# driskai/scenario_gym

Measured on AMD Instinct MI355X. Metric: entity-steps/sec (batched rollout), higher is better.
Workload: dtype f64

## Files before the change

### scenario_gym_amd/csrc/sgym_control.hpp

```cpp
#pragma once

namespace sg {

struct CtlLds { double ctrl[9][64]; double seg[5][64]; };

template <bool FAST, bool RIDERS = false>
__device__ __forceinline__ void control_body_l(CtlLds &lds ,
                                               const unsigned qblock ,
                                               const Params &p, double timestep, int n_steps, int first, int k0,
                                               const double *actions , double *tab, int row0, int metrics)
{
    const int lane = threadIdx.x;
    const size_t q = (size_t)qblock * 64 + lane;
    const int ent_raw = p.ctl_ent[q];
    const bool active = ent_raw >= 0;
    const uint32_t ent = active ? (uint32_t)ent_raw : 0u;
    const uint32_t r = ent / (uint32_t)p.EP;
    const LanePtr st(p.stat + (size_t)(ent >> 6) * (ST_COUNT * 64), (ent & 63) * 8u);
    const LanePtr dy(p.dyn + (size_t)(ent >> 6) * ((size_t)p.FROWS * 64), (ent & 63) * 8u);
    const int64_t meta = fld<int64_t>(st, ST_META);
    const int kind = active ? (int)(meta & 0xff) : SG_KIND_NONE;
    const double min_t = fld(st, ST_MIN_T), bl = fld(st, ST_BL);
    const bool is_ego = active && (int)(ent - r * (uint32_t)p.EP) == p.sstat[r].ego;
#pragma unroll
    for (int c = 0; c < 9; ++c) lds.ctrl[c][lane] = fld(st, ST_CTRL + c);
    const size_t NP = (size_t)p.n_ctl_pad;
    double *cst = p.ctl_state + q;

    double pose[6], t, prev_t;
    double m_avg, m_max, m_t;
    bool present;
    CtrlState cs;
    if (first) {
        const sg_scenario_state &sd = p.sdyn[r];
        t = sd.t;
        prev_t = sd.prev_t;
        m_avg = sd.ego_avg_speed; m_max = sd.ego_max_speed; m_t = sd.avg_t;
        present = fld<uint64_t>(dy, SG_F_PRESENT) != 0;
#pragma unroll
        for (int c = 0; c < 6; ++c) pose[c] = fld(dy, SG_F_POSE + c);
        cs.speed = fld(dy, SG_F_CTRL + 0); cs.e_lon_prev = fld(dy, SG_F_CTRL + 1);
        cs.e_lat_prev = fld(dy, SG_F_CTRL + 2); cs.e_lon_int = fld(dy, SG_F_CTRL + 3);
    } else {
#pragma unroll
        for (int c = 0; c < 6; ++c) pose[c] = cst[(CS_POSE + c) * NP];
        present = cst[CS_PRESENT * NP] != 0.0;
        cs.speed = cst[(CS_CTRL + 0) * NP]; cs.e_lon_prev = cst[(CS_CTRL + 1) * NP];
        cs.e_lat_prev = cst[(CS_CTRL + 2) * NP]; cs.e_lon_int = cst[(CS_CTRL + 3) * NP];
        t = cst[CS_T * NP];
        prev_t = cst[CS_PREV_T * NP];
        m_avg = cst[(CS_METRIC + 0) * NP]; m_max = cst[(CS_METRIC + 1) * NP]; m_t = cst[(CS_METRIC + 2) * NP];
    }
    if (!active) present = false;

    Table T;
    {
        const double *kn = p.knots + fld<int64_t>(st, ST_KNOT_OFF) * 7;
        T.x = kn; T.xs = 7; T.y = kn + 1; T.ys = 7; T.cs = 1;
        T.n = active ? (int)(meta >> 32) : 0;
    }
    double seg_hi;
    int seg_cur;
    double sgr[5] = {0.0, 0.0, 0.0, 0.0, 0.0};
    auto seg_publish = [&](const Segment &S) {
        lds.seg[0][lane] = S.x_lo;
        lds.seg[1][lane] = S.ylo[0]; lds.seg[2][lane] = S.ylo[1];
        lds.seg[3][lane] = S.sl[0]; lds.seg[4][lane] = S.sl[1];
        if (FAST) { sgr[0] = S.x_lo; sgr[1] = S.ylo[0]; sgr[2] = S.ylo[1]; sgr[3] = S.sl[0]; sgr[4] = S.sl[1]; }
        seg_hi = S.x_hi;
        seg_cur = S.cur;
    };
    {
        Segment S;
        S.cur = seg_locate(T, t);
        seg_load(T, S);
        seg_publish(S);
    }
    double *out = tab + (q * (size_t)(p.tab_steps + 1) + (size_t)row0) * CT_W;
    double *out1 = out + (size_t)p.n_ctl_pad * ((size_t)(p.tab_steps + 1) * CT_W);
    double *out2 = out1 + (size_t)p.n_ctl_pad * ((size_t)(p.tab_steps + 1) * CT_W);
    const bool replay_lane = RIDERS && (kind == SG_KIND_REPLAY || kind == SG_KIND_AGENT_REPLAY);
    const double max_t = fld(st, ST_MAX_T);
    const bool is_static = (int)(meta >> 32) == 1;
    Table TR{};
    Segment SR{};
    if (RIDERS) {
        TR = lane_table(p, replay_lane ? kind : SG_KIND_NONE, p.sstat[r], (int)(ent - r * (uint32_t)p.EP), st);
        if (!replay_lane) TR.n = 0;
        SR.cur = seg_locate(TR, t);
        seg_load(TR, SR);
    }
    sg_loads_done();
    const bool fast_kind = FAST && !p.ctl_general && sg_all(!active || (kind == SG_KIND_AGENT_PID && bl > 0.0 && bl < 0x1p400));
    const RecipDiv rd_l(active ? bl : 1.0), rd_10(10.0);
    double cpr[9];
#pragma unroll
    for (int c = 0; c < 9; ++c) cpr[c] = FAST ? fld(st, ST_CTRL + c) : 0.0;
    sg_loads_done();

    for (int k = 0; k < n_steps; ++k) {
        const double *Kp = SG_TRIG;
        if (!FAST) asm volatile("" : "+s"(Kp));
        ConstTbl K = (ConstTbl)Kp;
        const double next_t = t + timestep;
        const double state_dt = t - prev_t;
        const double dt = next_t - t;
        if (FAST && fast_kind && sg_all(!active || (present && !(next_t > seg_hi) && __builtin_fabs(pose[3]) < 1.0e5))) {
            const double dq = next_t - sgr[0];
            const double tx = sgr[3] * dq + sgr[1], ty = sgr[4] * dq + sgr[2];
            double sin_h, cos_h;
            sg_sincos_core(pose[3], sin_h, cos_h, K);
            const double e0 = tx - pose[0], e1 = ty - pose[1];
            const double e_lon = cos_h * e0 + sin_h * e1;
            const double e_lat = -sin_h * e0 + cos_h * e1;
            const double speed0 = cs.speed;
            const double g_mid = 1.0 - rd_10.div(0.9 * (speed0 - 5.0));
            const double gain = (speed0 > 5.0 && speed0 <= 15) ? g_mid : (speed0 > 15 ? 0.1 : 1.0);
            const RecipDiv rd(state_dt);
            const double d_lat = e_lat - cs.e_lat_prev, d_lon = e_lon - cs.e_lon_prev;
            const double e_lat_D = rd.div(d_lat);
            const double kp = cpr[SG_C_STEER_KP] * gain, kd = cpr[SG_C_STEER_KD] * gain;
            double steer = kp * e_lat + kd * e_lat_D;
            const double e_lon_D = rd.div(d_lon);
            const double e_lon_I = cs.e_lon_int + e_lon * state_dt;
            double accel = cpr[SG_C_ACCEL_KP] * e_lon + cpr[SG_C_ACCEL_KD] * e_lon_D + cpr[SG_C_ACCEL_KI] * e_lon_I;
            accel = __builtin_fabs(e_lon) > 0.1 ? accel : 0.0;
            const double max_steer = cpr[SG_C_MAX_STEER], max_accel = cpr[SG_C_MAX_ACCEL];
            const double max_speed = cpr[SG_C_MAX_SPEED], allow_rev = cpr[SG_C_ALLOW_REVERSE];
            accel = __builtin_fmin(__builtin_fmax(accel, -max_accel), max_accel);
            steer = __builtin_fmin(__builtin_fmax(steer, -max_steer), max_steer);
            const double dxs = speed0 * cos_h, dys = speed0 * sin_h;
            double tan_s = sg_tan_poly(steer, K);
            const bool steep = !(__builtin_fabs(steer) < 0.67434);
            if (sg_any(steep & active)) {
                double s2, c2;
                sg_sincos_core(steer, s2, c2, K);
                tan_s = steep ? s2 / c2 : tan_s;
            }
            const double hnum = speed0 * tan_s;
            const double dh = hnum == 0.0 ? hnum : rd_l.div(hnum);
            const double nx = pose[0] + dxs * dt, ny = pose[1] + dys * dt, nh = pose[3] + dh * dt;
            double nspeed = speed0 + accel * dt;
            nspeed = allow_rev == 0.0 ? __builtin_fmax(0.0, nspeed) : nspeed;
            nspeed = max_speed == max_speed ? __builtin_fmin(max_speed, nspeed) : nspeed;
            bool ok = rd.safe(d_lat) & rd.safe(d_lon) & (__builtin_fabs(steer) < 1.0e5) & (rd_l.safe(hnum) | (hnum == 0.0));
            double n_avg = m_avg, n_max = m_max, n_mt = m_t;
            if (metrics) {
                const RecipDiv rdt(dt), rnt(next_t);
                const double ax = nx - pose[0], ay = ny - pose[1];
                const double az = pose[2] - pose[2];
                const double speed = sg_norm3(rdt.div(ax), rdt.div(ay), 0.0);
                const double w = rnt.div(m_t);
                n_avg = m_avg + (1.0 - w) * (speed - m_avg);
                n_max = __builtin_fmax(speed, m_max);
                n_mt = next_t;
                ok = ok & (!is_ego | (rdt.safe(ax) & rdt.safe(ay) & rnt.safe(m_t) & (dt > 0.0) & (az == 0.0)));
            }
            if (sg_all(!active || ok)) {
                cs.e_lat_prev = e_lat; cs.e_lon_prev = e_lon; cs.e_lon_int = e_lon_I; cs.speed = nspeed;
                pose[0] = nx; pose[1] = ny; pose[3] = nh;
                if (is_ego) { m_avg = n_avg; m_max = n_max; m_t = n_mt; }
                prev_t = t;
                t = next_t;
                *reinterpret_cast<double4 *>(out + (size_t)k * CT_W) = make_double4(pose[0], pose[1], pose[3], cs.speed);
                *reinterpret_cast<double4 *>(out1 + (size_t)k * CT_W) = make_double4(cs.e_lon_prev, cs.e_lat_prev, cs.e_lon_int, 0.0);
                if (is_ego && metrics) *reinterpret_cast<double4 *>(out2 + (size_t)k * CT_W) = make_double4(m_avg, m_max, m_t, 0.0);
                continue;
            }
        }
        double act_a = 0.0, act_s = 0.0;
        if (kind == SG_KIND_AGENT_VEHICLE && actions) {
            const double *a = actions + ((size_t)(k0 + k) * p.R + r) * 2;
            act_a = a[0];
            act_s = a[1];
        }
        if (next_t > seg_hi) {
            Segment S;
            S.x_hi = seg_hi;
            S.cur = seg_cur;
            seg_advance(T, S, next_t);
            seg_publish(S);
            sg_loads_done();
        }
        double np_[6];
        const double dq = next_t - lds.seg[0][lane];
        np_[0] = lds.seg[3][lane] * dq + lds.seg[1][lane];
        np_[1] = lds.seg[4][lane] * dq + lds.seg[2][lane];
        bool npres = false;
        if (RIDERS && replay_lane) {
            if (next_t > SR.x_hi) { seg_advance(TR, SR, next_t); sg_loads_done(); }
            const double dqr = next_t - SR.x_lo;
#pragma unroll
            for (int c = 0; c < 6; ++c) np_[c] = SR.sl[c] * dqr + SR.ylo[c];
            npres = kind == SG_KIND_REPLAY ? (p.persist || is_static || (next_t >= min_t && next_t <= max_t))
                                           : (present || min_t >= t);
        } else if (present) {
            npres = true;
            const double tx = np_[0], ty = np_[1];
#pragma unroll
            for (int c = 0; c < 6; ++c) np_[c] = pose[c];
            double sin_h, cos_h;
            sg_sincos(pose[3], sin_h, cos_h, K);
            auto cp = [&](int q) -> double { return lds.ctrl[q][lane]; };
            if (kind == SG_KIND_AGENT_PID)
                pid_step(cs, cp, bl, state_dt, dt, tx, ty, sin_h, cos_h, np_, K);
            else
                vehicle_step(cs, cp, bl, dt, act_a, act_s, sin_h, cos_h, np_, K);
        } else if (active && min_t >= t) {
            npres = true;
            Segment S;
            S.cur = seg_cur;
            seg_load(T, S);
            sg_loads_done();
            const double dqs = next_t - S.x_lo;
#pragma unroll
            for (int c = 0; c < 6; ++c) np_[c] = S.sl[c] * dqs + S.ylo[c];
        }
        if (is_ego && npres && metrics) {
            double prev[6];
            if (!present) {
                own_position_extrap(T.x, T.n, t, prev);
                sg_loads_done();
            } else {
#pragma unroll
                for (int c = 0; c < 6; ++c) prev[c] = pose[c];
            }
            const double v0 = (np_[0] - prev[0]) / dt, v1 = (np_[1] - prev[1]) / dt, v2 = (np_[2] - prev[2]) / dt;
            const double speed = sg_norm3(v0, v1, v2);
            const double w = m_t / next_t;
            m_avg += (1.0 - w) * (speed - m_avg);
            m_t = next_t;
            m_max = __builtin_fmax(speed, m_max);
        }
        present = npres;
        if (npres) {
#pragma unroll
            for (int c = 0; c < 6; ++c) pose[c] = np_[c];
        }
        prev_t = t;
        t = next_t;
        *reinterpret_cast<double4 *>(out + (size_t)k * CT_W) = make_double4(pose[0], pose[1], pose[3], cs.speed);
        *reinterpret_cast<double4 *>(out1 + (size_t)k * CT_W) = make_double4(cs.e_lon_prev, cs.e_lat_prev, cs.e_lon_int, 0.0);
        if (is_ego && metrics) *reinterpret_cast<double4 *>(out2 + (size_t)k * CT_W) = make_double4(m_avg, m_max, m_t, 0.0);
        if (RIDERS) *reinterpret_cast<double4 *>(out2 + (size_t)k * CT_W) = make_double4(pose[2], pose[4], pose[5], present ? 1.0 : 0.0);
    }
#pragma unroll
    for (int c = 0; c < 6; ++c) cst[(CS_POSE + c) * NP] = pose[c];
    cst[CS_PRESENT * NP] = present ? 1.0 : 0.0;
    cst[(CS_CTRL + 0) * NP] = cs.speed; cst[(CS_CTRL + 1) * NP] = cs.e_lon_prev;
    cst[(CS_CTRL + 2) * NP] = cs.e_lat_prev; cst[(CS_CTRL + 3) * NP] = cs.e_lon_int;
    cst[CS_T * NP] = t;
    cst[CS_PREV_T * NP] = prev_t;
    cst[(CS_METRIC + 0) * NP] = m_avg; cst[(CS_METRIC + 1) * NP] = m_max; cst[(CS_METRIC + 2) * NP] = m_t;
}

template <bool FAST, bool RIDERS = false>
__device__ __forceinline__ void control_body(const Params &p, double timestep, int n_steps, int first, int k0,
                                             const double *actions , double *tab, int row0, int metrics)
{
    __shared__ CtlLds lds;
    control_body_l<FAST, RIDERS>(lds, blockIdx.x, p, timestep, n_steps, first, k0, actions, tab, row0, metrics);
}

#ifdef SG_UNIT_CTL
static __global__ __launch_bounds__(64, SG_CTL_WAVES) void control_kernel(Params p, double timestep, int n_steps, int first, int k0,
                                                     const double *actions , double *tab, int row0, int metrics)
{
    control_body<false>(p, timestep, n_steps, first, k0, actions, tab, row0, metrics);
}
#endif
#ifdef SG_UNIT_CTL
static __global__ __launch_bounds__(64, 2) void control_kernel_riders(Params p, double timestep, int n_steps, int first, int k0,
                                                               const double *actions , double *tab, int row0, int metrics)
{
    control_body<false, true>(p, timestep, n_steps, first, k0, actions, tab, row0, 0);
}
#endif
#ifdef SG_UNIT_CTL
static __global__ __launch_bounds__(64, 1) void control_kernel_fast(Params p, double timestep, int n_steps, int first, int k0,
                                                             const double *actions , double *tab, int row0, int metrics)
{
#ifdef SG_CTL_SETPRIO
    __builtin_amdgcn_s_setprio(3);
#endif
    control_body<true>(p, timestep, n_steps, first, k0, actions, tab, row0, metrics);
}
#endif

}
```

### scenario_gym_amd/csrc/sgym_core.hpp

```cpp
#pragma once

namespace sg {

enum {
    ST_BW = 0, ST_BL, ST_BCX, ST_BCY,
    ST_MIN_T, ST_MAX_T,
    ST_KNOT_OFF,
    ST_META,
    ST_ROUTE,
    ST_CTL,
    ST_CTRL,
    NCTRL_ROWS = 13,
    ST_COUNT = ST_CTRL + NCTRL_ROWS
};
constexpr uint32_t ROW = 512;

struct ScenStatic {
    double t0, length;
    int64_t grid_off;
    int32_t grid_n, ego;
};

struct RoadNet { double x0, y0, inv_cell; int32_t nx, ny; int64_t cell_base; };
struct RoadCand { int32_t poly; uint32_t edge_off; uint16_t n_edges; uint8_t ref_sel, ref_inside; };
struct RoadIndex {
    const RoadNet *nets;
    const int32_t *net_of_scen;
    const uint16_t *cells;
    const uint32_t *cell_off;
    const RoadCand *cand;
    const int32_t *cand_edges;
    const double *edges;
    const uint32_t *poly_layers;
    const uint32_t *net_flags;
    const int64_t *imp_off;
    const double *imp_edges;
    const double *imp_aux;
    const double *imp_m;
    int32_t n_nets;
};

struct Params {
    int R, E, EP;
    int persist;
    unsigned term_mask;
    int rec_cap, ev_cap;
    const double *stat;
    const ScenStatic *sstat;
    const double *knots;
    const double *grid_t;
    double *grid_y;
    double *dyn;
    sg_scenario_state *sdyn;
    sg_event *events;
    double *ev_pose;
    double *ev_hpose;
    double *rec_t, *rec_pose;
    const double *routes;
    const double *gon;
    int WV, FROWS;
    sg_social_force sf;
    const int32_t *ctl_ent;
    double *ctl_state;
    int n_ctl_pad;
    const double *ext_pose;
    int32_t *rss_state, *rss_code, *rss_seen;
    double *rss_safe;
    double *rssq;
    int32_t *rssq_n;
    int32_t rssq_cap;
    const unsigned char *reset_mask;
    const RoadIndex *road;
    int ctl_general;
    int ped_serial;
    int quiet;
    int tab_steps;
    int noise_mode;
    double noise_std_lon, noise_std_lat;
    const double *noise_normals;
    long long noise_len;
    unsigned long long noise_seed;
    int ped_behaviour;
    int n_ped_models;
    const double *ped_models;
    const int32_t *model_of;
#ifdef SG_PHASE_TIMERS
    unsigned long long *phase_cycles;
#endif
};

enum { PM_BEHAVIOUR = 0, PM_SF = 1, PM_STD_LON = 13, PM_STD_LAT = 14, PM_W = 16 };
static_assert(sizeof(sg_social_force) == 12 * sizeof(double), "sg_social_force is twelve doubles");

enum { CT_X = 0, CT_Y, CT_H, CT_SPEED, CT_W = 4, CT_ELON = 0, CT_ELAT, CT_EINT, CT_MAVG = 0, CT_MMAX, CT_MT, CT_PLANES = 3 };
enum { CS_POSE = 0, CS_PRESENT = 6, CS_CTRL = 7, CS_T = 11, CS_PREV_T = 12, CS_METRIC = 13, CS_COUNT = 16 };

#define SG_GLOBAL __attribute__((address_space(1)))
struct LanePtr {
    SG_GLOBAL char *a[3];
    __device__ __forceinline__ LanePtr(const double *blk, uint32_t voff)
    {
        a[0] = (SG_GLOBAL char *)(reinterpret_cast<char *>(const_cast<double *>(blk)) + voff);
        a[1] = a[0] + 8 * ROW;
        a[2] = a[0] + 16 * ROW;
        asm("" : "+v"(a[1]), "+v"(a[2]));
    }
};
template <typename T = double>
__device__ __forceinline__ T fld(const LanePtr &lp, int f)
{
    const int b = f < 24 ? f >> 3 : 2;
    return *reinterpret_cast<SG_GLOBAL const T *>(lp.a[b] + (f - 8 * b) * (int)ROW);
}
template <typename T>
__device__ __forceinline__ void stf(const LanePtr &lp, int f, T v)
{
    const int b = f < 24 ? f >> 3 : 2;
    *reinterpret_cast<SG_GLOBAL T *>(lp.a[b] + (f - 8 * b) * (int)ROW) = v;
}

__device__ __forceinline__ double sg_norm3(double a, double b, double c)
{
    return __builtin_sqrt(__builtin_fma(c, c, __builtin_fma(b, b, a * a)));
}
__device__ __forceinline__ double sg_norm2(double a, double b)
{
    return __builtin_sqrt(__builtin_fma(b, b, a * a));
}

__device__ __noinline__ double2 sg_sincos_slow(double x)
{
    return make_double2(sin(x), cos(x));
}

static __constant__ double SG_TRIG[48] = {
    6.36619772367581382433e-01,
    1.57079632673412561417e+00,
    6.07710050630396597660e-11,
    2.02226624879595063154e-21,
    -1.66666666666666324348e-01, 8.33333333332248946124e-03, -1.98412698298579493134e-04,
    2.75573137070700676789e-06, -2.50507602534068634195e-08, 1.58969099521155010221e-10,
    4.16666666666666019037e-02, -1.38888888888741095749e-03, 2.48015872894767294178e-05,
    -2.75573143513906633035e-07, 2.08757232129817482790e-09, -1.13596475577881948265e-11,
    3.33333333333334091986e-01, 1.33333333333201242699e-01, 5.39682539762260521377e-02,
    2.18694882948595424599e-02, 8.86323982359930005737e-03, 3.59207910759131235356e-03,
    1.45620945432529025516e-03, 5.88041240820264096874e-04, 2.46463134818469906812e-04,
    7.81794442939557092300e-05, 7.14072491382608190305e-05, -1.85586374855275456654e-05,
    2.59073051863633712884e-05, 0.0, 0.0, 0.0,
    3.33333333333329318027e-01, -1.99999999998764832476e-01, 1.42857142725034663711e-01, -1.11111104054623557880e-01,
    9.09088713343650656196e-02, -7.69187620504482999495e-02, 6.66107313738753120669e-02, -5.83357013379057348645e-02,
    4.97687799461593236017e-02, -3.65315727442169155270e-02, 1.62858201153657823623e-02, 0.0, 0.0, 0.0, 0.0, 0.0,
};

typedef const __attribute__((address_space(4))) double *ConstTbl;

__device__ __forceinline__ void sg_sincos_core(double x, double &s, double &c, ConstTbl K);

__device__ __forceinline__ void sg_sincos(double x, double &s, double &c, ConstTbl K = (ConstTbl)SG_TRIG)
{
    if (!(__builtin_fabs(x) < 1.0e5)) {
        double2 sc = sg_sincos_slow(x);
        s = sc.x;
        c = sc.y;
        return;
    }
    sg_sincos_core(x, s, c, K);
}

__device__ __forceinline__ void sg_sincos_core(double x, double &s, double &c, ConstTbl K)
{
    double fn = __builtin_rint(x * K[0]);
    int n = (int)fn;
    double t = x - fn * K[1];
    double w = fn * K[2];
    double r = t - w;
    w = fn * K[3] - ((t - r) - w);
    double y0 = r - w;
    double y1 = (r - y0) - w;
    double z = y0 * y0;
    double v = z * y0;
    double rs = K[5] + z * (K[6] + z * (K[7] + z * (K[8] + z * K[9])));
    double ks = y0 - ((z * (0.5 * y1 - v * rs) - y1) - v * K[4]);
    double rc = z * (K[10] + z * (K[11] + z * (K[12] + z * (K[13] + z * (K[14] + z * K[15])))));
    double ay = __builtin_fabs(y0);
    uint64_t qb = ((uint64_t)__double_as_longlong(ay) - ((uint64_t)0x00200000 << 32)) & 0xFFFFFFFF00000000ULL;
    double qx = ay > 0.78125 ? 0.28125 : __longlong_as_double((long long)qb);
    qx = ay < 0.3 ? 0.0 : qx;
    double hz = 0.5 * z - qx;
    double a = 1.0 - qx;
    double kc = a - (hz - (z * rc - y0 * y1));
    double ss = (n & 1) ? kc : ks;
    double cc = (n & 1) ? ks : kc;
    s = (n & 2) ? -ss : ss;
    c = ((n + 1) & 2) ? -cc : cc;
}

__device__ __forceinline__ double sg_tan_poly(double x, ConstTbl K)
{
    ConstTbl T = K + 16;
    double z = x * x;
    double w = z * z;
    double r = T[1] + w * (T[3] + w * (T[5] + w * (T[7] + w * (T[9] + w * T[11]))));
    double v = z * (T[2] + w * (T[4] + w * (T[6] + w * (T[8] + w * (T[10] + w * T[12])))));
    double s = z * x;
    r = z * (s * (r + v));
    r = r + T[0] * s;
    return x + r;
}

__device__ __forceinline__ double sg_tan(double x, ConstTbl K)
{
    if (!(__builtin_fabs(x) < 0.67434)) {
        double s, c;
        sg_sincos(x, s, c, K);
        return s / c;
    }
    return sg_tan_poly(x, K);
}

#define SG_TRIG32_ERR 4.0e-6f
__device__ __forceinline__ void sg_sincos_f32(double h, float &s, float &c)
{
    if (!(__builtin_fabs(h) < 1.0e5)) {
        double2 sc = sg_sincos_slow(h);
        s = (float)sc.x;
        c = (float)sc.y;
        return;
    }
    const double rev = h * 1.59154943091895345554e-01;
    const float f = (float)(rev - __builtin_rint(rev));
    s = __builtin_amdgcn_sinf(f);
    c = __builtin_amdgcn_cosf(f);
}

__device__ __forceinline__ double sg_pred(double x)
{
    long long b = __double_as_longlong(x);
    if (x > 0.0) return __longlong_as_double(b - 1);
    if (x < 0.0) return __longlong_as_double(b + 1);
    return -4.9406564584124654e-324;
}

__device__ __forceinline__ bool sg_any(bool p) { return __builtin_amdgcn_ballot_w64(p) != 0; }
__device__ __forceinline__ bool sg_all(bool p) { return __builtin_amdgcn_ballot_w64(!p) == 0; }

__device__ __forceinline__ double shfl_d(double v, int src) { return __shfl(v, src, 64); }

__device__ __forceinline__ void sg_loads_done() { __builtin_amdgcn_s_waitcnt(0x0F70); }
__device__ __forceinline__ void sg_lgkm_done() { __builtin_amdgcn_s_waitcnt(0xC07F); }

struct RecipDiv {
    double b, r;
    bool ok;
    __device__ __forceinline__ explicit RecipDiv(double den) : b(den)
    {
        double ab = __builtin_fabs(den);
        ok = ab > 0x1p-500 && ab < 0x1p500;
        double r0 = __builtin_amdgcn_rcp(den);
        double e0 = __builtin_fma(-den, r0, 1.0);
        double r1 = __builtin_fma(r0, e0, r0);
        double e1 = __builtin_fma(-den, r1, 1.0);
        r = __builtin_fma(r1, e1, r1);
    }
    __device__ __forceinline__ bool safe(double a) const
    {
        uint32_t e = ((uint32_t)__double2hiint(a) >> 20) & 0x7ffu;
        return ok & (((e - 64u) < 1920u) | (__double_as_longlong(a) == 0));
    }
    __device__ __forceinline__ double div(double a) const
    {
        double q0 = a * r;
        double e = __builtin_fma(-b, q0, a);
        return __builtin_fma(e, r, q0);
    }
};

struct Table {
    const double *x;
    const double *y;
    int n;
    int xs, ys, cs;
    __device__ __forceinline__ double X(int i) const { return x[(size_t)i * xs]; }
    __device__ __forceinline__ double Y(int i, int c) const { return y[(size_t)i * ys + (size_t)c * cs]; }
};

struct Segment {
    double x_lo, x_hi;
    double ylo[6], sl[6];
    int cur;
};

__device__ __forceinline__ void seg_load(const Table &T, Segment &S)
{
    const int n = T.n, cur = S.cur;
    if (n <= 0) {
        S.x_lo = 0.0;
        S.x_hi = __builtin_inf();
#pragma unroll
        for (int c = 0; c < 6; ++c) { S.ylo[c] = 0.0; S.sl[c] = 0.0; }
        return;
    }
    if (cur == 0 || cur >= n || n == 1) {
        int row = cur == 0 ? 0 : n - 1;
        double x0 = T.X(row);
        S.x_lo = x0;
        S.x_hi = (cur == 0 && n > 1) ? sg_pred(x0) : __builtin_inf();
#pragma unroll
        for (int c = 0; c < 6; ++c) { S.ylo[c] = T.Y(row, c); S.sl[c] = 0.0; }
        return;
    }
    double x_lo = T.X(cur - 1), x_hi = T.X(cur);
    S.x_lo = x_lo;
    S.x_hi = x_hi;
    double dx = x_hi - x_lo;
#pragma unroll
    for (int c = 0; c < 6; ++c) {
        double a = T.Y(cur - 1, c), b = T.Y(cur, c);
        S.ylo[c] = a;
        S.sl[c] = (b - a) / dx;
    }
}

__device__ __forceinline__ int seg_locate(const Table &T, double t)
{
    const int n = T.n;
    if (n <= 1) return 0;
    if (t < T.X(0)) return 0;
    if (t > T.X(n - 1)) return n;
    int lo = 0, hi = n;
    while (lo < hi) {
        int mid = (lo + hi) >> 1;
        if (T.X(mid) < t) lo = mid + 1; else hi = mid;
    }
    return lo < 1 ? 1 : (lo > n - 1 ? n - 1 : lo);
}

__device__ __forceinline__ void seg_advance(const Table &T, Segment &S, double t)
{
    if (t > S.x_hi) {
        int cur = S.cur == 0 ? 1 : S.cur;
        while (cur <= T.n - 1 && T.X(cur) < t) ++cur;
        S.cur = cur;
        seg_load(T, S);
    }
}

__device__ __forceinline__ void own_position_extrap(const double *kn, int n, double t, double (&out)[6])
{
    if (n == 1) {
        double x_lo = kn[0];
#pragma unroll
        for (int c = 0; c < 6; ++c) {
            double slope = kn[1 + c] - kn[1 + c];
            out[c] = slope * (t - x_lo) + kn[1 + c];
        }
        return;
    }
    int lo = 0, hi = n;
    while (lo < hi) {
        int mid = (lo + hi) >> 1;
        if (kn[(size_t)mid * 7] < t) lo = mid + 1; else hi = mid;
    }
    int idx = lo < 1 ? 1 : (lo > n - 1 ? n - 1 : lo);
    const double *a = kn + (size_t)(idx - 1) * 7, *b = kn + (size_t)idx * 7;
#pragma unroll
    for (int c = 0; c < 6; ++c) {
        double slope = (b[1 + c] - a[1 + c]) / (b[0] - a[0]);
        out[c] = slope * (t - a[0]) + a[1 + c];
    }
}

__device__ __forceinline__ void sg_corners(double x, double y, double s, double c, double W, double L,
                                           double cx, double cy, double *o)
{
    double pxm = cx - 0.5 * L, pxp = cx + 0.5 * L, pyp = cy + 0.5 * W, pym = cy - 0.5 * W;
    double ns = -s;
    o[0] = x + (pxm * c + pyp * ns); o[1] = y + (pxm * s + pyp * c);
    o[2] = x + (pxp * c + pyp * ns); o[3] = y + (pxp * s + pyp * c);
    o[4] = x + (pxp * c + pym * ns); o[5] = y + (pxp * s + pym * c);
    o[6] = x + (pxm * c + pym * ns); o[7] = y + (pxm * s + pym * c);
}

__device__ __forceinline__ bool sg_sat_pass(const double *P, const double *Q)
{
    double o = (P[4] - P[0]) * (P[7] - P[3]) - (P[5] - P[1]) * (P[6] - P[2]);
    bool sep = false;
#pragma unroll
    for (int i = 0; i < 4; ++i) {
        int j = (i + 1) & 3;
        double ax = P[2 * i], ay = P[2 * i + 1];
        double ex = P[2 * j] - ax, ey = P[2 * j + 1] - ay;
        bool all_out = true;
#pragma unroll
        for (int k = 0; k < 4; ++k) {
            double cr = ex * (Q[2 * k + 1] - ay) - ey * (Q[2 * k] - ax);
            bool out = o > 0 ? (cr < 0) : (cr > 0);
            all_out = all_out && out;
        }
        sep = sep || all_out;
    }
    return sep;
}
__device__ __forceinline__ bool sg_quads_intersect(const double *A, const double *B)
{
    return !(sg_sat_pass(A, B) || sg_sat_pass(B, A));
}

typedef float v2f __attribute__((ext_vector_type(2)));
typedef double v2d __attribute__((ext_vector_type(2)));
typedef float v4f __attribute__((ext_vector_type(4)));

template <int NS, bool PED, bool CROWD = false, bool ROADTAB = false>
struct TileLds {
    float cx[NS], cy[NS];
    float2 sc[NS];
    float2 cen[NS];
    unsigned long long xtab[64][NS / 64], ytab[64][NS / 64];
    double cor[8][NS > 64 ? NS : 2];
    float2 half[NS];
    int last[NS];
    int vote[4][8];
    double ctrl[PED ? 4 : 9][NS];
    double boxwl[2][NS];
    double px[PED ? NS : 1], py[PED ? NS : 1], vx[PED ? NS : 1], vy[PED ? NS : 1];
    double ox[PED ? NS : 1], oy[PED ? NS : 1], stp[PED ? NS : 1];
    unsigned char isped[PED ? NS : 1];
    double sx[CROWD ? NS : 1], sy[CROWD ? NS : 1], ss[CROWD ? NS : 1];
    double r2hi[CROWD ? NS : 1], r2lo[CROWD ? NS : 1];
    uint32_t nq[CROWD ? 8 : 1][CROWD ? NS : 1];
    double ego_m[CROWD ? 3 : 1];
    unsigned long long ego_last[CROWD ? (NS + 63) / 64 : 1];
    int ego_nev[2];
    static constexpr bool GON = CROWD && NS != 128;
    double gon[GON ? 128 : 1];
    static constexpr bool ROAD_TAB = ROADTAB;
    static constexpr int ROAD_EDGES = 64;
    double road_tab[ROADTAB ? ROAD_EDGES * 5 : 1];
    double road_m;
    RoadNet road_net;
    int road_info[4];

    static constexpr int SLOTS = NS;
    static constexpr int SCRATCH_BYTES = NS * 40 + 64 * (NS > 64 ? NS : 2);
    static constexpr int PAIR_CAP = NS > 64 ? 320 : 128;
    __device__ __forceinline__ char *wave_scratch(int wave) { return reinterpret_cast<char *>(cx) + wave * (PAIR_CAP * 20); }
};
static_assert(TileLds<256, true>::PAIR_CAP * 20 * 4 <= TileLds<256, true>::SCRATCH_BYTES, "pair scratch");
static_assert(TileLds<128, true>::PAIR_CAP * 20 * 2 <= TileLds<128, true>::SCRATCH_BYTES, "pair scratch");
static_assert(TileLds<64, true>::PAIR_CAP * 20 <= TileLds<64, true>::SCRATCH_BYTES, "pair scratch");
typedef TileLds<256, true> TileLdsWide;
static_assert(offsetof(TileLdsWide, half) == TileLdsWide::SCRATCH_BYTES, "collision scratch is contiguous");

}
```

### scenario_gym_amd/csrc/sgym_queue.hpp

```cpp
#pragma once

namespace sg {

enum { Q_TICKET = 0, Q_HEAD = 1, Q_ERR = 2, Q_ITEMS_DONE = 3, Q_CTL_CLAIMED = 4, Q_STATE_WORDS = 8 };
constexpr int Q_SEATS = 1 << 14;
enum { Q_ERR_CTL_WAIT = 1, Q_ERR_BLOCK_WAIT = 2, Q_ERR_RING_WAIT = 3 };
constexpr int Q_MAX_CHUNKS = 255;
constexpr int Q_PROG_STRIDE = 32;

struct TabQueue {
    unsigned *state;
    unsigned *ctl_prog;
    unsigned *blk_prog;
    unsigned *chunk_cnt;
    unsigned *seats;
    long long defer_ticks;
    double *tab;
    size_t buf_doubles;
    const double *actions;
    unsigned *trace;
    unsigned long long *times;
    long long timeout_ticks;
    int n_chunks, n_buf, nblk, n_ctl_waves;
    int nap;
    int lag_prio;
    int handoff;
    int k0[Q_MAX_CHUNKS + 1];
};

__device__ __forceinline__ unsigned q_peek(const unsigned *w)
{
    return (unsigned)__builtin_amdgcn_readfirstlane((int)__hip_atomic_load(w, __ATOMIC_RELAXED, __HIP_MEMORY_SCOPE_AGENT));
}

__device__ __forceinline__ bool q_wait_ge(const unsigned *w, unsigned want, const TabQueue &tq, unsigned code)
{
    if (q_peek(w) >= want) return true;
    const long long t0 = wall_clock64();
    for (int spin = 0;; ++spin) {
        if (spin < 4) __builtin_amdgcn_s_sleep(16);
        else if (spin < 12) __builtin_amdgcn_s_sleep(112);
        else {
            const int n = min(tq.nap, 1 << min((spin - 12) >> 2, 6));
            for (int i = 0; i < n; ++i) __builtin_amdgcn_s_sleep(127);
        }
        if (q_peek(w) >= want) return true;
        if ((spin & 7) == 7 && q_peek(tq.state + Q_ERR) != 0) return false;
        if (wall_clock64() - t0 > tq.timeout_ticks) {
            if (threadIdx.x == 0) atomicCAS(tq.state + Q_ERR, 0u, code);
            return false;
        }
    }
}

__device__ __forceinline__ void q_acquire()
{
    __builtin_amdgcn_fence(__ATOMIC_ACQUIRE, "agent");
    asm volatile("s_dcache_inv\n\ts_waitcnt lgkmcnt(0)" ::: "memory");
}

__device__ __forceinline__ void q_release()
{
    asm volatile("s_waitcnt vmcnt(0)" ::: "memory");
    __builtin_amdgcn_fence(__ATOMIC_RELEASE, "agent");
    asm volatile("s_waitcnt vmcnt(0)" ::: "memory");
}

template <int G>
__device__ __forceinline__ void q_handoff_writethrough(const Params &p, unsigned b, int lane)
{
    asm volatile("s_waitcnt vmcnt(0)" ::: "memory");
    typedef SG_GLOBAL unsigned long long gu64;
    constexpr int FR = SG_F_COLL + 1;
    gu64 *rows = (gu64 *)(p.dyn + (size_t)b * ((size_t)FR * 64)) + lane;
    unsigned long long v[FR];
#pragma unroll
    for (int f = 0; f < FR; ++f) v[f] = __hip_atomic_load(rows + f * 64, __ATOMIC_RELAXED, __HIP_MEMORY_SCOPE_AGENT);
#pragma unroll
    for (int f = 0; f < FR; ++f) __hip_atomic_store(rows + f * 64, v[f], __ATOMIC_RELAXED, __HIP_MEMORY_SCOPE_AGENT);
    static_assert(sizeof(sg_scenario_state) % 8 == 0, "scenario records are copied in 8-byte words");
    constexpr int SW = (int)(sizeof(sg_scenario_state) / 8);
    const int gl = (int)b * 64 + lane, r = gl / G, slot = gl & (G - 1);
    if (r < p.R) {
        gu64 *sd = (gu64 *)(p.sdyn + r);
        for (int w = slot; w < SW; w += G) {
            const unsigned long long v = __hip_atomic_load(sd + w, __ATOMIC_RELAXED, __HIP_MEMORY_SCOPE_AGENT);
            __hip_atomic_store(sd + w, v, __ATOMIC_RELAXED, __HIP_MEMORY_SCOPE_AGENT);
        }
    }
    asm volatile("s_waitcnt vmcnt(0)" ::: "memory");
}

template <int G, unsigned F>
__device__ __forceinline__ void tabq_body(const Params &p, double timestep, int force, const TabQueue &tq)
{
    constexpr bool RSS = (F & V_RSS) != 0;
    using Tile = typename Variant<G, 1, F>::Lds;
    static_assert(sizeof(Tile) >= sizeof(CtlLds), "the pre-pass role lays its LDS over the tile");
    __shared__ Tile lds;
    __shared__ typename std::conditional<RSS, RssQueue, char>::type rssq_lds;
    const int lane = threadIdx.x;
    unsigned ticket = ~0u;
    {
        const unsigned hw = (unsigned)__builtin_amdgcn_s_getreg((4 << 0) | (0 << 6) | (31 << 11));
        const unsigned xcc = (unsigned)__builtin_amdgcn_s_getreg((20 << 0) | (0 << 6) | (3 << 11));
        const unsigned seat = ((xcc & 15u) << 10) | (((hw >> 13) & 7u) << 7) | (((hw >> 12) & 1u) << 6) | (((hw >> 8) & 15u) << 2) | ((hw >> 4) & 3u);
        unsigned rank = 0;
        if (lane == 0) {
            atomicAdd(tq.state + Q_TICKET, 1u);
            rank = atomicAdd(tq.seats + seat, 1u);
        }
        rank = (unsigned)__builtin_amdgcn_readfirstlane((int)rank);
        bool claim = rank == 0 && q_peek(tq.state + Q_CTL_CLAIMED) < (unsigned)tq.n_ctl_waves;
        if (rank != 0) {
            const long long t0 = wall_clock64();
            while (q_peek(tq.state + Q_CTL_CLAIMED) < (unsigned)tq.n_ctl_waves) {
                if (wall_clock64() - t0 > tq.defer_ticks) { claim = true; break; }
                __builtin_amdgcn_s_sleep(8);
            }
        }
        if (claim) {
            unsigned idx = 0;
            if (lane == 0) idx = atomicAdd(tq.state + Q_CTL_CLAIMED, 1u);
            idx = (unsigned)__builtin_amdgcn_readfirstlane((int)idx);
            if (idx < (unsigned)tq.n_ctl_waves) ticket = idx;
        }
    }

    if (ticket < (unsigned)tq.n_ctl_waves) {
        __builtin_amdgcn_s_setprio(3);
        CtlLds &cl = *reinterpret_cast<CtlLds *>(&lds);
        for (int c = 0; c < tq.n_chunks; ++c) {
            if (c >= tq.n_buf && !q_wait_ge(tq.chunk_cnt + (c - tq.n_buf), (unsigned)tq.nblk, tq, Q_ERR_RING_WAIT)) break;
            control_body_l<true>(cl, ticket, p, timestep, tq.k0[c + 1] - tq.k0[c], c == 0, tq.k0[c], tq.actions,
                                 tq.tab + (size_t)(c % tq.n_buf) * tq.buf_doubles, 0, RSS ? 0 : 1);
            q_release();
            if (tq.times && lane == 0) tq.times[(size_t)tq.n_chunks * tq.nblk * 4 + (size_t)ticket * tq.n_chunks + c] = wall_clock64();
            if (lane == 0) __hip_atomic_store(tq.ctl_prog + ticket * Q_PROG_STRIDE, (unsigned)(c + 1), __ATOMIC_RELAXED, __HIP_MEMORY_SCOPE_AGENT);
        }
        __builtin_amdgcn_s_setprio(0);
        if (q_peek(tq.state + Q_ERR) != 0) return;
    }

    const unsigned n_items = (unsigned)tq.n_chunks * (unsigned)tq.nblk;
    unsigned done_b = ~0u, done_c = 0;
    for (;;) {
        unsigned item = 0;
        if (lane == 0) {
            if (done_b != ~0u) {
                __hip_atomic_store(tq.blk_prog + done_b, done_c + 1, __ATOMIC_RELAXED, __HIP_MEMORY_SCOPE_AGENT);
                if (tq.n_buf < tq.n_chunks) atomicAdd(tq.chunk_cnt + done_c, 1u);
                atomicAdd(tq.state + Q_ITEMS_DONE, 1u);
            }
            item = atomicAdd(tq.state + Q_HEAD, 1u);
        }
        item = (unsigned)__builtin_amdgcn_readfirstlane((int)item);
        done_b = ~0u;
        if (item >= n_items) break;
        const unsigned c = item / (unsigned)tq.nblk, b = item - c * (unsigned)tq.nblk;
        auto trace = [&](unsigned stage) {
            if (tq.trace && lane == 0) __hip_atomic_store(tq.trace + b, (c << 8) | stage, __ATOMIC_RELAXED, __HIP_MEMORY_SCOPE_AGENT);
        };
        trace(1);
        auto stamp = [&](int k) {
            if (tq.times && lane == 0) tq.times[(size_t)item * 4 + k] = wall_clock64();
        };
        stamp(0);
        if (tq.lag_prio) __builtin_amdgcn_s_setprio(0);
        const bool behind = c != 0 && q_peek(tq.blk_prog + b) < c;
        bool ok = c == 0 || q_wait_ge(tq.blk_prog + b, c, tq, Q_ERR_BLOCK_WAIT);
        {
            const LanePtr st(p.stat + (size_t)b * (ST_COUNT * 64), (uint32_t)lane * 8u);
            const int64_t cq = fld<int64_t>(st, ST_CTL);
            uint64_t m = __ballot(cq >= 0);
            while (m && ok) {
                const int l = __builtin_ctzll(m);
                m &= m - 1;
                const unsigned w = (unsigned)__builtin_amdgcn_readlane((int)(uint32_t)cq, l) >> 6;
                ok = q_wait_ge(tq.ctl_prog + w * Q_PROG_STRIDE, c + 1, tq, Q_ERR_CTL_WAIT);
            }
        }
        if (!ok) break;
        if (tq.lag_prio && behind) {
            if (tq.lag_prio == 1) __builtin_amdgcn_s_setprio(1);
            else __builtin_amdgcn_s_setprio(2);
        }
        trace(2);
        q_acquire();
        trace(3);
        stamp(1);
        const double *tab = tq.tab + (size_t)(c % (unsigned)tq.n_buf) * tq.buf_doubles;
        const int gl = (int)b * 64 + lane, r_raw = gl / G;
        const bool in_range = r_raw < p.R;
        const int r = in_range ? r_raw : p.R - 1;
        const int ev_before = p.ev_cap > 0 ? min(p.sdyn[r].n_events, p.ev_cap) : 0;
        rollout_body_l<G, 1, F>(lds, p, timestep, tq.k0[c + 1] - tq.k0[c], 0, force, nullptr, tab, SliceArgs{}, b);
        trace(4);
        stamp(2);
        if (RSS) {
            asm volatile("s_waitcnt vmcnt(0)" ::: "memory");
            rss_lines_block(p, (RssQueueLds)&rssq_lds, (size_t)b);
        }
        if (!RSS && p.ev_cap > 0) {
            asm volatile("s_waitcnt vmcnt(0)" ::: "memory");
            const int ev_after = in_range ? min(p.sdyn[r].n_events, p.ev_cap) : 0;
            if (ev_after > ev_before) {
                int64_t ectl;
                const bool from_tab = ego_table_column(p, r, ectl);
                for (int i = ev_before + (gl & (G - 1)); i < ev_after; i += G) event_take_table_pose(p, r, i, tab, from_tab, ectl);
            }
        }
        trace(5);
        if (RSS) {
            asm volatile("s_waitcnt vmcnt(0)" ::: "memory");
            typedef SG_GLOBAL int gi32;
            typedef SG_GLOBAL unsigned long long gu64;
            const size_t idx = (size_t)b * 64 + lane;
            gi32 *sw = (gi32 *)(p.rss_state + idx), *cw = (gi32 *)(p.rss_code + idx);
            gu64 *fw = (gu64 *)(p.rss_safe + idx * 2);
            const int v0 = __hip_atomic_load(sw, __ATOMIC_RELAXED, __HIP_MEMORY_SCOPE_AGENT);
            const int v1 = __hip_atomic_load(cw, __ATOMIC_RELAXED, __HIP_MEMORY_SCOPE_AGENT);
            const unsigned long long v2 = __hip_atomic_load(fw, __ATOMIC_RELAXED, __HIP_MEMORY_SCOPE_AGENT);
            const unsigned long long v3 = __hip_atomic_load(fw + 1, __ATOMIC_RELAXED, __HIP_MEMORY_SCOPE_AGENT);
            __hip_atomic_store(sw, v0, __ATOMIC_RELAXED, __HIP_MEMORY_SCOPE_AGENT);
            __hip_atomic_store(cw, v1, __ATOMIC_RELAXED, __HIP_MEMORY_SCOPE_AGENT);
            __hip_atomic_store(fw, v2, __ATOMIC_RELAXED, __HIP_MEMORY_SCOPE_AGENT);
            __hip_atomic_store(fw + 1, v3, __ATOMIC_RELAXED, __HIP_MEMORY_SCOPE_AGENT);
            const int glr = (int)b * 64 + lane;
            if ((glr & (G - 1)) == 0 && glr / G < p.R) {
                gi32 *nw = (gi32 *)(p.rss_seen + glr / G);
                const int v4 = __hip_atomic_load(nw, __ATOMIC_RELAXED, __HIP_MEMORY_SCOPE_AGENT);
                __hip_atomic_store(nw, v4, __ATOMIC_RELAXED, __HIP_MEMORY_SCOPE_AGENT);
            }
        }
        if (tq.handoff == 1) q_handoff_writethrough<G>(p, b, lane);
        else q_release();
        trace(6);
        stamp(3);
        done_b = b;
        done_c = c;
    }
    if (lane == 0 && done_b != ~0u) {
        __hip_atomic_store(tq.blk_prog + done_b, done_c + 1, __ATOMIC_RELAXED, __HIP_MEMORY_SCOPE_AGENT);
        if (tq.n_buf < tq.n_chunks) atomicAdd(tq.chunk_cnt + done_c, 1u);
        atomicAdd(tq.state + Q_ITEMS_DONE, 1u);
    }
}

template <int G>
__global__ __launch_bounds__(64, SG_TAB_WAVES) __attribute__((amdgpu_num_vgpr(SG_TAB_VGPR))) void rollout_kernel_tabq(
    Params p, double timestep, int force, TabQueue tq)
{
    tabq_body<G, V_TAB | V_HAST>(p, timestep, force, tq);
}
template <int G>
__global__ __launch_bounds__(64, SG_PLANAR_WAVES) __attribute__((amdgpu_num_vgpr(SG_PLANAR_VGPR))) void rollout_kernel_tabq_planar(
    Params p, double timestep, int force, TabQueue tq)
{
    tabq_body<G, V_TAB | V_HAST | V_PLANAR>(p, timestep, force, tq);
}

template <int G>
__global__ __launch_bounds__(64, SG_WAVES_PER_SIMD) void rollout_kernel_rss_tabq(Params p, double timestep, int force, TabQueue tq)
{
    tabq_body<G, V_RSS | V_CTAB>(p, timestep, force, tq);
}

}
```

Baseline: 148.8 billion.

## Hand-schedule fast PID control step with inlined trig, reciprocals and compile-time metrics

Rewrites the fast path of the per-entity PID controller step as a manually interleaved instruction schedule. Sincos, tan polynomial, the three reciprocal refinements and the sqrt used for the metric speed are inlined so independent chains overlap, and metrics become a template parameter so the branch is resolved at compile time. Empty asm barriers pin some values in registers. The aim is to shorten the serial dependency latency of the per-step loop on the control wavefronts, which bound the pipeline. The cost is much more fragile code, more register pressure, and metrics now computed speculatively even for non-ego lanes.

After: 150.6 billion, median of 5. 1.01x the previous value.

```diff
diff --git a/scenario_gym_amd/csrc/sgym_control.hpp b/scenario_gym_amd/csrc/sgym_control.hpp
--- a/scenario_gym_amd/csrc/sgym_control.hpp
+++ b/scenario_gym_amd/csrc/sgym_control.hpp
@@ -4,12 +4,13 @@
 
 struct CtlLds { double ctrl[9][64]; double seg[5][64]; };
 
-template <bool FAST, bool RIDERS = false>
+template <bool FAST, bool RIDERS = false, int METRICS = -1>
 __device__ __forceinline__ void control_body_l(CtlLds &lds ,
                                                const unsigned qblock ,
                                                const Params &p, double timestep, int n_steps, int first, int k0,
-                                               const double *actions , double *tab, int row0, int metrics)
-{
+                                               const double *actions , double *tab, int row0, int metrics_arg)
+{
+    const int metrics = METRICS < 0 ? metrics_arg : METRICS;
     const int lane = threadIdx.x;
     const size_t q = (size_t)qblock * 64 + lane;
     const int ent_raw = p.ctl_ent[q];
@@ -105,61 +106,165 @@
         const double next_t = t + timestep;
         const double state_dt = t - prev_t;
         const double dt = next_t - t;
-        if (FAST && fast_kind && sg_all(!active || (present && !(next_t > seg_hi) && __builtin_fabs(pose[3]) < 1.0e5))) {
-            const double dq = next_t - sgr[0];
-            const double tx = sgr[3] * dq + sgr[1], ty = sgr[4] * dq + sgr[2];
-            double sin_h, cos_h;
-            sg_sincos_core(pose[3], sin_h, cos_h, K);
-            const double e0 = tx - pose[0], e1 = ty - pose[1];
-            const double e_lon = cos_h * e0 + sin_h * e1;
-            const double e_lat = -sin_h * e0 + cos_h * e1;
-            const double speed0 = cs.speed;
-            const double g_mid = 1.0 - rd_10.div(0.9 * (speed0 - 5.0));
-            const double gain = (speed0 > 5.0 && speed0 <= 15) ? g_mid : (speed0 > 15 ? 0.1 : 1.0);
-            const RecipDiv rd(state_dt);
-            const double d_lat = e_lat - cs.e_lat_prev, d_lon = e_lon - cs.e_lon_prev;
-            const double e_lat_D = rd.div(d_lat);
-            const double kp = cpr[SG_C_STEER_KP] * gain, kd = cpr[SG_C_STEER_KD] * gain;
-            double steer = kp * e_lat + kd * e_lat_D;
-            const double e_lon_D = rd.div(d_lon);
-            const double e_lon_I = cs.e_lon_int + e_lon * state_dt;
-            double accel = cpr[SG_C_ACCEL_KP] * e_lon + cpr[SG_C_ACCEL_KD] * e_lon_D + cpr[SG_C_ACCEL_KI] * e_lon_I;
-            accel = __builtin_fabs(e_lon) > 0.1 ? accel : 0.0;
+        if (FAST && fast_kind && sg_all(!active | (present & !(next_t > seg_hi) & (__builtin_fabs(pose[3]) < 1.0e5)))) {
+            const double hd = pose[3], speed0 = cs.speed;
             const double max_steer = cpr[SG_C_MAX_STEER], max_accel = cpr[SG_C_MAX_ACCEL];
             const double max_speed = cpr[SG_C_MAX_SPEED], allow_rev = cpr[SG_C_ALLOW_REVERSE];
-            accel = __builtin_fmin(__builtin_fmax(accel, -max_accel), max_accel);
-            steer = __builtin_fmin(__builtin_fmax(steer, -max_steer), max_steer);
+            const double fn0 = hd * K[0];
+            const double dq = next_t - sgr[0];
+            double ra = __builtin_amdgcn_rcp(state_dt), rb = __builtin_amdgcn_rcp(dt), rn = __builtin_amdgcn_rcp(next_t);
+            const double fn = __builtin_rint(fn0);
+            const double txm = sgr[3] * dq, tym = sgr[4] * dq;
+            const double g1 = speed0 - 5.0;
+            const double t1 = fn * K[1], w1 = fn * K[2], w3 = fn * K[3];
+            double ea = __builtin_fma(-state_dt, ra, 1.0);
+            const double tt = hd - t1;
+            double eb = __builtin_fma(-dt, rb, 1.0), en = __builtin_fma(-next_t, rn, 1.0);
+            const double tx = txm + sgr[1];
+            const double r_ = tt - w1;
+            const double ty = tym + sgr[2];
+            const double g2 = 0.9 * g1;
+            ra = __builtin_fma(ra, ea, ra);
+            const double tr = tt - r_;
+            rb = __builtin_fma(rb, eb, rb); rn = __builtin_fma(rn, en, rn);
+            const double e0 = tx - pose[0];
+            const double trw = tr - w1;
+            const double e1 = ty - pose[1];
+            const double g3q = g2 * rd_10.r;
+            ea = __builtin_fma(-state_dt, ra, 1.0);
+            const double w2 = w3 - trw;
+            eb = __builtin_fma(-dt, rb, 1.0); en = __builtin_fma(-next_t, rn, 1.0);
+            const double g3e = __builtin_fma(-rd_10.b, g3q, g2);
+            const double y0 = r_ - w2;
+            ra = __builtin_fma(ra, ea, ra); rb = __builtin_fma(rb, eb, rb); rn = __builtin_fma(rn, en, rn);
+            const RecipDiv rd(state_dt, ra), rdt(dt, rb), rnt(next_t, rn);
+            const double ry = r_ - y0, z = y0 * y0;
+            const double g3 = __builtin_fma(g3e, rd_10.r, g3q);
+            const double ay0 = __builtin_fabs(y0);
+            const uint64_t qb = ((uint64_t)__double_as_longlong(ay0) - ((uint64_t)0x00200000 << 32)) & 0xFFFFFFFF00000000ULL;
+            const double y1 = ry - w2, v = z * y0;
+            double rs = z * K[9], rc = z * K[15];
+            const double wq0 = m_t * rnt.r;
+            const double g_mid = 1.0 - g3;
+            rs = K[8] + rs; rc = K[14] + rc;
+            const double wqe = __builtin_fma(-next_t, wq0, m_t);
+            const double gain = (speed0 > 5.0 && speed0 <= 15) ? g_mid : (speed0 > 15 ? 0.1 : 1.0);
+            rs = z * rs; rc = z * rc;
+            const double w = __builtin_fma(wqe, rnt.r, wq0);
+            const double kp = cpr[SG_C_STEER_KP] * gain;
+            rs = K[7] + rs; rc = K[13] + rc;
+            const double omw = 1.0 - w;
+            const double kd = cpr[SG_C_STEER_KD] * gain;
+            rs = z * rs; rc = z * rc;
+            double qx = ay0 > 0.78125 ? 0.28125 : __longlong_as_double((long long)qb);
+            rs = K[6] + rs; rc = K[12] + rc;
+            qx = ay0 < 0.3 ? 0.0 : qx;
+            const double hy = 0.5 * y1;
+            rs = z * rs; rc = z * rc;
+            const double yy = y0 * y1, vk4 = v * K[4];
+            rs = K[5] + rs; rc = K[11] + rc;
+            const double hz = 0.5 * z - qx, qa = 1.0 - qx;
+            const double vrs = v * rs; rc = z * rc;
+            const int n = (int)fn;
+            const double s1 = hy - vrs; rc = K[10] + rc;
+            const double az = pose[2] - pose[2];
+            const double s2 = z * s1; rc = z * rc;
+            bool ok_m = rnt.safe(m_t) & (dt > 0.0) & (az == 0.0);
+            const double s3 = s2 - y1, zrc = z * rc;
+            const double s4 = s3 - vk4, c1 = zrc - yy;
+            const double ks = y0 - s4, c2 = hz - c1;
+            const double kc = qa - c2;
+            const double ss = (n & 1) ? kc : ks, cc = (n & 1) ? ks : kc;
+            const double sin_h = (n & 2) ? -ss : ss, cos_h = ((n + 1) & 2) ? -cc : cc;
+            const double m1 = -sin_h * e0, m2 = cos_h * e1, l1 = cos_h * e0, l2 = sin_h * e1;
             const double dxs = speed0 * cos_h, dys = speed0 * sin_h;
-            double tan_s = sg_tan_poly(steer, K);
+            const double e_lat = m1 + m2, e_lon = l1 + l2;
+            const double dxdt = dxs * dt, dydt = dys * dt;
+            const double d_lat = e_lat - cs.e_lat_prev, pk = kp * e_lat, d_lon = e_lon - cs.e_lon_prev;
+            const double nx = pose[0] + dxdt, ny = pose[1] + dydt;
+            const double lq0 = d_lat * rd.r, eli = e_lon * state_dt;
+            const double ax = nx - pose[0], ay = ny - pose[1];
+            const double lqe = __builtin_fma(-state_dt, lq0, d_lat), nq0 = d_lon * rd.r;
+            const double e_lon_I = cs.e_lon_int + eli;
+            const double vx0 = ax * rdt.r, vy0 = ay * rdt.r;
+            const double e_lat_D = __builtin_fma(lqe, rd.r, lq0), nqe = __builtin_fma(-state_dt, nq0, d_lon);
+            const double vxe = __builtin_fma(-dt, vx0, ax), vye = __builtin_fma(-dt, vy0, ay);
+            bool ok = rd.safe(d_lat) & rd.safe(d_lon);
+            const double dk = kd * e_lat_D, e_lon_D = __builtin_fma(nqe, rd.r, nq0), ak = cpr[SG_C_ACCEL_KP] * e_lon;
+            const double vx = __builtin_fma(vxe, rdt.r, vx0), vy = __builtin_fma(vye, rdt.r, vy0);
+            double steer = pk + dk;
+            const double ad = cpr[SG_C_ACCEL_KD] * e_lon_D, ai = cpr[SG_C_ACCEL_KI] * e_lon_I;
+            double sq = vx * vx;
+            ok_m = ok_m & rdt.safe(ax) & rdt.safe(ay);
+            steer = __builtin_fmax(steer, -max_steer);
+            double accel = ak + ad;
+            sq = __builtin_fma(vy, vy, sq);
+            steer = __builtin_fmin(steer, max_steer);
+            accel = accel + ai;
+            sq = __builtin_fma(0.0, 0.0, sq);
+            const double tz = steer * steer;
+            accel = __builtin_fabs(e_lon) > 0.1 ? accel : 0.0;
+            const bool q_small = sq < 0x1p-767;
+            const double qs = __builtin_ldexp(sq, q_small ? 256 : 0);
+            const double tw = tz * tz, ts = tz * steer;
+            accel = __builtin_fmax(accel, -max_accel);
+            const double qy = __builtin_amdgcn_rsq(qs);
+            ConstTbl T = K + 16;
+            double tr_ = tw * T[11], tv = tw * T[12];
+            accel = __builtin_fmin(accel, max_accel);
+            ok = ok & (__builtin_fabs(steer) < 1.0e5);
+            tr_ = T[9] + tr_; tv = T[10] + tv;
+            const double adt = accel * dt;
+            double qg = qs * qy, qh = qy * 0.5;
+            tr_ = tw * tr_; tv = tw * tv;
+            double nspeed = speed0 + adt;
+            const double qr = __builtin_fma(-qh, qg, 0.5);
+            tr_ = T[7] + tr_; tv = T[8] + tv;
+            nspeed = allow_rev == 0.0 ? __builtin_fmax(0.0, nspeed) : nspeed;
+            qg = __builtin_fma(qg, qr, qg); qh = __builtin_fma(qh, qr, qh);
+            tr_ = tw * tr_; tv = tw * tv;
+            nspeed = max_speed == max_speed ? __builtin_fmin(max_speed, nspeed) : nspeed;
+            double qd = __builtin_fma(-qg, qg, qs);
+            tr_ = T[5] + tr_; tv = T[6] + tv;
+            qg = __builtin_fma(qd, qh, qg);
+            tr_ = tw * tr_; tv = tw * tv;
+            qd = __builtin_fma(-qg, qg, qs);
+            tr_ = T[3] + tr_; tv = T[4] + tv;
+            qg = __builtin_fma(qd, qh, qg);
+            tr_ = tw * tr_; tv = tw * tv;
+            qg = __builtin_ldexp(qg, q_small ? -128 : 0);
+            tr_ = T[1] + tr_; tv = T[2] + tv;
+            const double speed = __builtin_amdgcn_class(qs, 0x260) ? qs : qg;
+            tv = tz * tv;
+            const double t0s = T[0] * ts;
+            const double dsp = speed - m_avg, mx = __builtin_fmax(speed, m_max);
+            const double trv = tr_ + tv;
+            const double dm = omw * dsp;
+            const double tsr = ts * trv;
+            const double avg = m_avg + dm;
+            const double tzr = tz * tsr;
+            double n_avg = (metrics && is_ego) ? avg : m_avg, n_max = (metrics && is_ego) ? mx : m_max, n_mt = (metrics && is_ego) ? next_t : m_t;
+            const double trr = tzr + t0s;
+            double tan_s = steer + trr;
+            if (metrics) ok = ok & (!is_ego | ok_m);
+            double c_int = e_lon_I, c_speed = nspeed;
+            unsigned c_ok = ok;
+            if (metrics) asm volatile("" : "+v"(c_int), "+v"(c_speed), "+v"(n_avg), "+v"(n_max), "+v"(c_ok), "+v"(tan_s));
+            else asm volatile("" : "+v"(c_int), "+v"(c_speed), "+v"(c_ok), "+v"(tan_s));
             const bool steep = !(__builtin_fabs(steer) < 0.67434);
             if (sg_any(steep & active)) {
-                double s2, c2;
-                sg_sincos_core(steer, s2, c2, K);
-                tan_s = steep ? s2 / c2 : tan_s;
+                double s2_, c2_;
+                sg_sincos_core(steer, s2_, c2_, K);
+                tan_s = steep ? s2_ / c2_ : tan_s;
             }
             const double hnum = speed0 * tan_s;
             const double dh = hnum == 0.0 ? hnum : rd_l.div(hnum);
-            const double nx = pose[0] + dxs * dt, ny = pose[1] + dys * dt, nh = pose[3] + dh * dt;
-            double nspeed = speed0 + accel * dt;
-            nspeed = allow_rev == 0.0 ? __builtin_fmax(0.0, nspeed) : nspeed;
-            nspeed = max_speed == max_speed ? __builtin_fmin(max_speed, nspeed) : nspeed;
-            bool ok = rd.safe(d_lat) & rd.safe(d_lon) & (__builtin_fabs(steer) < 1.0e5) & (rd_l.safe(hnum) | (hnum == 0.0));
-            double n_avg = m_avg, n_max = m_max, n_mt = m_t;
-            if (metrics) {
-                const RecipDiv rdt(dt), rnt(next_t);
-                const double ax = nx - pose[0], ay = ny - pose[1];
-                const double az = pose[2] - pose[2];
-                const double speed = sg_norm3(rdt.div(ax), rdt.div(ay), 0.0);
-                const double w = rnt.div(m_t);
-                n_avg = m_avg + (1.0 - w) * (speed - m_avg);
-                n_max = __builtin_fmax(speed, m_max);
-                n_mt = next_t;
-                ok = ok & (!is_ego | (rdt.safe(ax) & rdt.safe(ay) & rnt.safe(m_t) & (dt > 0.0) & (az == 0.0)));
-            }
-            if (sg_all(!active || ok)) {
-                cs.e_lat_prev = e_lat; cs.e_lon_prev = e_lon; cs.e_lon_int = e_lon_I; cs.speed = nspeed;
-                pose[0] = nx; pose[1] = ny; pose[3] = nh;
-                if (is_ego) { m_avg = n_avg; m_max = n_max; m_t = n_mt; }
+            const double c_h = hd + dh * dt;
+            ok = (c_ok != 0) & (rd_l.safe(hnum) | (hnum == 0.0));
+            if (sg_all(!active | ok)) {
+                cs.e_lat_prev = e_lat; cs.e_lon_prev = e_lon; cs.e_lon_int = c_int; cs.speed = c_speed;
+                pose[0] = nx; pose[1] = ny; pose[3] = c_h;
+                m_avg = n_avg; m_max = n_max; m_t = n_mt;
                 prev_t = t;
                 t = next_t;
                 *reinterpret_cast<double4 *>(out + (size_t)k * CT_W) = make_double4(pose[0], pose[1], pose[3], cs.speed);
@@ -254,12 +359,12 @@
     cst[(CS_METRIC + 0) * NP] = m_avg; cst[(CS_METRIC + 1) * NP] = m_max; cst[(CS_METRIC + 2) * NP] = m_t;
 }
 
-template <bool FAST, bool RIDERS = false>
+template <bool FAST, bool RIDERS = false, int METRICS = -1>
 __device__ __forceinline__ void control_body(const Params &p, double timestep, int n_steps, int first, int k0,
                                              const double *actions , double *tab, int row0, int metrics)
 {
     __shared__ CtlLds lds;
-    control_body_l<FAST, RIDERS>(lds, blockIdx.x, p, timestep, n_steps, first, k0, actions, tab, row0, metrics);
+    control_body_l<FAST, RIDERS, METRICS>(lds, blockIdx.x, p, timestep, n_steps, first, k0, actions, tab, row0, metrics);
 }
 
 #ifdef SG_UNIT_CTL
@@ -283,7 +388,9 @@
 #ifdef SG_CTL_SETPRIO
     __builtin_amdgcn_s_setprio(3);
 #endif
-    control_body<true>(p, timestep, n_steps, first, k0, actions, tab, row0, metrics);
+    __shared__ CtlLds lds;
+    if (metrics) control_body_l<true, false, 1>(lds, blockIdx.x, p, timestep, n_steps, first, k0, actions, tab, row0, 1);
+    else control_body_l<true, false, 0>(lds, blockIdx.x, p, timestep, n_steps, first, k0, actions, tab, row0, 0);
 }
 #endif
 
diff --git a/scenario_gym_amd/csrc/sgym_core.hpp b/scenario_gym_amd/csrc/sgym_core.hpp
--- a/scenario_gym_amd/csrc/sgym_core.hpp
+++ b/scenario_gym_amd/csrc/sgym_core.hpp
@@ -262,6 +262,11 @@
         double e1 = __builtin_fma(-den, r1, 1.0);
         r = __builtin_fma(r1, e1, r1);
     }
+    __device__ __forceinline__ RecipDiv(double den, double refined) : b(den), r(refined)
+    {
+        double ab = __builtin_fabs(den);
+        ok = ab > 0x1p-500 && ab < 0x1p500;
+    }
     __device__ __forceinline__ bool safe(double a) const
     {
         uint32_t e = ((uint32_t)__double2hiint(a) >> 20) & 0x7ffu;
diff --git a/scenario_gym_amd/csrc/sgym_queue.hpp b/scenario_gym_amd/csrc/sgym_queue.hpp
--- a/scenario_gym_amd/csrc/sgym_queue.hpp
+++ b/scenario_gym_amd/csrc/sgym_queue.hpp
@@ -132,8 +132,8 @@
         CtlLds &cl = *reinterpret_cast<CtlLds *>(&lds);
         for (int c = 0; c < tq.n_chunks; ++c) {
             if (c >= tq.n_buf && !q_wait_ge(tq.chunk_cnt + (c - tq.n_buf), (unsigned)tq.nblk, tq, Q_ERR_RING_WAIT)) break;
-            control_body_l<true>(cl, ticket, p, timestep, tq.k0[c + 1] - tq.k0[c], c == 0, tq.k0[c], tq.actions,
-                                 tq.tab + (size_t)(c % tq.n_buf) * tq.buf_doubles, 0, RSS ? 0 : 1);
+            control_body_l<true, false, RSS ? 0 : 1>(cl, ticket, p, timestep, tq.k0[c + 1] - tq.k0[c], c == 0, tq.k0[c], tq.actions,
+                                                     tq.tab + (size_t)(c % tq.n_buf) * tq.buf_doubles, 0, RSS ? 0 : 1);
             q_release();
             if (tq.times && lane == 0) tq.times[(size_t)tq.n_chunks * tq.nblk * 4 + (size_t)ticket * tq.n_chunks + c] = wall_clock64();
             if (lane == 0) __hip_atomic_store(tq.ctl_prog + ticket * Q_PROG_STRIDE, (unsigned)(c + 1), __ATOMIC_RELAXED, __HIP_MEMORY_SCOPE_AGENT);
```
